# tzjtatata/Myriad

Hardware: AMD Instinct MI355X
Metric: images/sec fine-tune step (Vicuna-7B + LoRA-style adapters, 224px) (higher is better)
Workload: dtype bf16

## Files before the change

### include/myriad_hip.h

```cpp
#ifndef MYRIAD_HIP_H
#define MYRIAD_HIP_H
#include <stdint.h>

#ifdef __cplusplus
extern "C" {
#endif

typedef struct ihipStream_t* mh_stream_t;

#define MH_OK 0
#define MH_ERR_ARG (-1)
#define MH_ERR_LAUNCH (-2)
#define MH_ERR_UNSUPPORTED (-3)

#define MH_GEMM_OUT_F32 1
#define MH_GEMM_GELU 2
#define MH_GEMM_REGSTAGE 4

int mh_gemm_bf16_nt(const void* A, int lda, const void* B, int ldb, void* C, int ldc, int M, int N, int K,
                    const float* bias, const float* residual, int ldr, int flags, float alpha, mh_stream_t s);

int mh_gemm_plan(int M, int N, int K, int flags, int* kernel, int* splits);

int mh_prof_start(int capacity, mh_stream_t s);
// ... 120 lines not shown

int mh_clamp_ce(const float* logits, long ldl, const long* labels, float* row_loss, void* dlogits_bf16, long ldd,
                int R, int V, float grad_scale, mh_stream_t s);
int mh_sum_f32(const float* x, float* out, long n, float scale, mh_stream_t s);
int mh_argmax_rows(const float* logits, long ldl, long* out, float* margin, int R, int V, int ban_id, mh_stream_t s);
int mh_argmax_pmax_rows(const float* logits, long ldl, long* out, float* margin, float* pmax, int R, int V, int ban_id,
                        float inv_temp, mh_stream_t s);
int mh_decode_record(const long* nxt, const float* margin, const float* pmax, float* rec, long* next_ids, int* step, int R,
                     mh_stream_t s);
int mh_decode_advance(const long* nxt, const float* margin, const float* pmax, float* rec, long* next_ids, int* step, int* pos,
                      int* kvlen, int R, mh_stream_t s);
int mh_sample_rows(const float* logits, long ldl, long* out, float* margin, float* pmax, int* kept, float* u_out, int R, int V,
                   int ban_id, const float* params, const unsigned long long* seed, const int* step, int t_add, mh_stream_t s);
int mh_repetition_penalty_rows(float* logits, long ldl, unsigned* seen, const long* prev_ids, int R, int V, const float* penalty,
                               mh_stream_t s);
int mh_decode_advance_kept(const long* nxt, const float* margin, const float* pmax, const int* kept, float* rec, long* next_ids,
                           int* step, int* pos, int* kvlen, int R, mh_stream_t s);
int mh_decode_advance_rows(const long* nxt, const float* margin, const float* pmax, float* rec, long* next_ids, int* step,
                           int* pos, int* kvlen, const int* live, int R, mh_stream_t s);
int mh_sample_rows_slots(const float* logits, long ldl, long* out, float* margin, float* pmax, int* kept, float* u_out, int R, int V,
                         const float* params, const unsigned long long* seed, const int* gen, const int* live, mh_stream_t s);
int mh_argmax_pmax_rows_slots(const float* logits, long ldl, long* out, float* margin, float* pmax, int R, int V, const float* params,
                              const int* gen, const int* live, mh_stream_t s);
int mh_repetition_penalty_rows_slots(float* logits, long ldl, unsigned* seen, const long* prev_ids, int R, int V, const float* penalty,
                                     const int* live, mh_stream_t s);
int mh_decode_advance_kept_rows(const long* nxt, const float* margin, const float* pmax, const int* kept, float* rec, long* next_ids,
                                int* step, int* pos, int* kvlen, int* gen, const int* live, int R, mh_stream_t s);
int mh_token_scores_rows(const float* logits, long ldl, const long* ids, const int* watch, float* out, long ldo, int R, int V,
                         const int* live, mh_stream_t s);

int mh_beam_topk(const float* logits, long ldl, const float* scores, float* part_s, int* part_i, float* out_s, int* out_i, int B,
                 int rpi, int nb, int V, int ban_id, int* pos, int* kvlen, int n_adv, mh_stream_t s);
int mh_beam_reorder_kv(void* const* caches, int L, int B, int nb, long T_cap, int C, const int* src, const int* lo, const int* hi,
                       mh_stream_t s);
int mh_beam_topk_items(const float* logits, long ldl, const float* scores, float* part_s, int* part_i, float* out_s, int* out_i, int G,
                       int nb, int V, const int* live, int* gen, const int* prm, int* pos, int* kvlen, mh_stream_t s);
int mh_beam_reorder_kv_items(void* const* caches, int L, int G, int nb, long T_cap, int C, const int* src, const int* lo,
                             const int* hi, const int* live, mh_stream_t s);
int mh_beam_sample_topk(const float* logits, long ldl, const float* scores, const unsigned* seen, float* part_k, float* part_a,
                        int* part_i, int* part_f, float* out_s, int* out_i, int* out_f, float* out_k, int B, int nb, int V,
                        int ban_id, int draw, const float* params, const unsigned long long* seed, int* step, int t_add, int* pos,
                        int* kvlen, int n_adv, mh_stream_t s);
int mh_beam_seen_update(unsigned* seen, const int* src, const long* ids, int B, int nb, int V, mh_stream_t s);

int mh_im2col_nhwc(const void* x, void* col, int B, int H, int W, int C, int kh, int kw, int pad, int Kpad,
                   mh_stream_t s);
int mh_col2im_nhwc(const void* dcol, float* dx, int B, int H, int W, int C, int kh, int kw, int pad, int Kpad,
                   mh_stream_t s);
int mh_relu_maxpool2_fwd(const void* y, int y_is_f32, long ldy, void* p, int B, int H, int W, int C, mh_stream_t s);
int mh_relu_maxpool2_bwd(const float* dp, const void* y, int y_is_f32, long ldy, void* dy, long lddy, int B, int H,
                         int W, int C, mh_stream_t s);
int mh_conv_pack_weight(const float* W, const float* bias, void* Wp, int Cout, int K, int Kpad, mh_stream_t s);
int mh_conv_unpack_grad(const float* dWp, float* dW, float* db, int Cout, int K, int Kpad, mh_stream_t s);

int mh_embed_gather(const void* table_bf16, const long* ids, const int* dst_rows, float* out, long n, int D, long ldo,
                    mh_stream_t s);
int mh_copy2d_f32(const float* src, long lds, float* dst, long ldd, long rows, int cols, int accumulate,
                  mh_stream_t s);
int mh_copy3d_f32(const float* src, long src_bstride, long lds, float* dst, long dst_bstride, long ldd, int nb,
                  long rows, int cols, int accumulate, mh_stream_t s);
int mh_gather_rows_f32_to_bf16(const float* src, long lds, const int* rows, void* dst, long n, int D, mh_stream_t s);
int mh_gather_rows_f32(const float* src, long lds, const int* rows, float* dst, long n, int D, mh_stream_t s);
int mh_gather_rows(const void* src, long lds, const int* rows, void* dst, long n, int D, int elem_bytes, mh_stream_t s);
int mh_expand_rows(const void* src, const int* inv, void* dst, long ldd, long M, int D, int elem_bytes, mh_stream_t s);
int mh_copy3d_bf16(const void* src, long src_bstride, long lds, void* dst, long dst_bstride, long ldd, int nb,
                   long rows, int cols, mh_stream_t s);
int mh_kv_append_bf16(const void* src, long ld_src, void* cache, long cache_bstride, long ld_cache, const int* pos_dev,
                      int B, int cols, mh_stream_t s);
int mh_rope_kv_append(void* qkv, long ld, int n_heads, int head_dim, const int* pos, const float* cos_tab,
                      const float* sin_tab, void* cache, long cache_bstride, long ld_cache, const int* pos_dev, int B,
                      mh_stream_t s);
int mh_add_i32(int* x, int n, int delta, mh_stream_t s);
long mh_gemv_pack_elems(int N, int K);
int mh_gemv_pack(const void* W, int ldb, int N, int K, void* out, mh_stream_t s);
int mh_gemv_packed(const void* A, int lda, const void* P, void* C, int ldc, int M, int N, int K, const float* bias,
                   const float* residual, int ldr, int out_f32, float alpha, mh_stream_t s);
int mh_gemv_packed_rmsnorm(const float* H, long ldh, const float* norm_w, float eps, const void* P, void* C, int ldc, int M,
                           int N, int K, const float* bias, const float* residual, int ldr, int out_f32, float alpha,
                           mh_stream_t s);
int mh_gemv_packed_silu(const void* gu, long ldgu, const void* P, void* C, int ldc, int M, int N, int K, const float* bias,
                        const float* residual, int ldr, int out_f32, float alpha, mh_stream_t s);
long mh_gemv_pack_fp8_elems(int N, int K);
int mh_gemv_pack_fp8(const void* W, int ldb, int N, int K, void* q_out, float* scale_out, mh_stream_t s);
int mh_gemv_packed_fp8(const void* A, int lda, const void* Q, const float* scale, void* C, int ldc, int M, int N, int K,
                       const float* bias, const float* residual, int ldr, int out_f32, float alpha, mh_stream_t s);
int mh_gemv_packed_fp8_rmsnorm(const float* H, long ldh, const float* norm_w, float eps, const void* Q, const float* scale,
                               void* C, int ldc, int M, int N, int K, const float* bias, const float* residual, int ldr,
                               int out_f32, float alpha, mh_stream_t s);
int mh_gemv_packed_fp8_silu(const void* gu, long ldgu, const void* Q, const float* scale, void* C, int ldc, int M, int N, int K,
                            const float* bias, const float* residual, int ldr, int out_f32, float alpha, mh_stream_t s);
long mh_gemv_pack_fp4_elems(int N, int K);
long mh_gemv_pack_fp4_scale_elems(int N, int K);
int mh_gemv_pack_fp4(const void* W, int ldb, int N, int K, void* q_out, void* scale_out, mh_stream_t s);
int mh_gemv_packed_fp4(const void* A, int lda, const void* Q, const void* scale, void* C, int ldc, int M, int N, int K,
                       const float* bias, const float* residual, int ldr, int out_f32, float alpha, mh_stream_t s);
int mh_gemv_packed_fp4_rmsnorm(const float* H, long ldh, const float* norm_w, float eps, const void* Q, const void* scale,
                               void* C, int ldc, int M, int N, int K, const float* bias, const float* residual, int ldr,
                               int out_f32, float alpha, mh_stream_t s);
int mh_gemv_packed_fp4_silu(const void* gu, long ldgu, const void* Q, const void* scale, void* C, int ldc, int M, int N, int K,
                            const float* bias, const float* residual, int ldr, int out_f32, float alpha, mh_stream_t s);
int mh_gemv_packed_wide(const void* A, int lda, const void* P, void* C, int ldc, int M, int N, int K, const float* bias,
                        const float* residual, int ldr, int out_f32, float alpha, mh_stream_t s);
int mh_gemv_packed_fp8_wide(const void* A, int lda, const void* Q, const float* scale, void* C, int ldc, int M, int N, int K,
                            const float* bias, const float* residual, int ldr, int out_f32, float alpha, mh_stream_t s);
int mh_gemv_packed_fp4_wide(const void* A, int lda, const void* Q, const void* scale, void* C, int ldc, int M, int N, int K,
                            const float* bias, const float* residual, int ldr, int out_f32, float alpha, mh_stream_t s);
// ... 123 lines not shown
```

### myriad_amd/csrc/common.h

```cpp
#pragma once
#include <hip/hip_runtime.h>
#include <stdint.h>

#define MH_OK 0
#define MH_ERR_ARG (-1)
#define MH_ERR_LAUNCH (-2)
#define MH_ERR_UNSUPPORTED (-3)

typedef unsigned short bf16_t;
typedef __attribute__((ext_vector_type(8))) short short8_t;
typedef __attribute__((ext_vector_type(4))) short short4_t;
typedef __attribute__((ext_vector_type(4))) float float4_t;
typedef __attribute__((ext_vector_type(16))) float float16_t;

#define MH_CHECK_LAUNCH()                                   \
  do {                                                      \
    hipError_t e__ = hipGetLastError();                     \
    if (e__ != hipSuccess) return MH_ERR_LAUNCH;            \
  } while (0)

#define MH_MAX_ALT_WS 4
struct MhScratch {
  float* ws;
  size_t bytes;
  float* alt[MH_MAX_ALT_WS];
  hipStream_t alt_stream[MH_MAX_ALT_WS];
};
extern MhScratch g_default_scratch;
extern MhScratch* g_scratch;

enum MhOpt {
  MH_OPT_SLAB_BF16 = 0,
  MH_OPT_GEMM_SKINNY,
  MH_OPT_SWIGLU_FUSED,
  MH_OPT_GELU_FUSED,
  MH_OPT_ATTN_BWD_SPLIT,
  MH_OPT_GEMM_ZERO_PAD,
  MH_OPT_GEMM256_IMPL,
  MH_OPT_LORA_NORM_FUSED,
  MH_OPT_ATTN_FULL,
  MH_OPT_LORA_WGRAD_MFMA,
  MH_OPT_GEMM_SKIP_PAD,
  MH_OPT_GEMM_SPLIT_XCD,
  MH_OPT_COUNT
};
int mh_opt(int id);

extern bool g_mh_prof_on;
void mh_prof_pre(hipStream_t s, int kernel, int M, int N, int K, int splits, int flags);
void mh_prof_post(hipStream_t s);

__device__ __forceinline__ float bf2f(bf16_t h) { return __uint_as_float(((unsigned)h) << 16); }

typedef __bf16 mh_bf2_t __attribute__((ext_vector_type(2)));
typedef float mh_f2_t __attribute__((ext_vector_type(2)));
__device__ __forceinline__ bf16_t f2bf_sw(float f) {
  unsigned u = __float_as_uint(f);
  if ((u & 0x7fffffffu) > 0x7f800000u) return (bf16_t)((u >> 16) | 0x40);
  u += 0x7fffu + ((u >> 16) & 1u);
  return (bf16_t)(u >> 16);
}
__device__ __forceinline__ bf16_t f2bf(float f) {
  const __bf16 b = (__bf16)f;
  return (bf16_t)__builtin_bit_cast(unsigned short, b);
}
__device__ __forceinline__ unsigned pack_bf2(float lo, float hi) {
  const mh_f2_t v = {lo, hi};
  const mh_bf2_t b = __builtin_convertvector(v, mh_bf2_t);
  return __builtin_bit_cast(unsigned, b);
}

__device__ __forceinline__ unsigned dropout_hash(unsigned long long seed, unsigned long long idx) {
  unsigned h = (unsigned)idx * 0x9E3779B1u + ((unsigned)seed ^ ((unsigned)(idx >> 32) * 0x85EBCA77u));
  h ^= (unsigned)(seed >> 32) & 0x7FFFFFFFu;
  h ^= h >> 16;
  h *= 0x85EBCA6Bu;
  h ^= h >> 13;
  h *= 0xC2B2AE35u;
  h ^= h >> 16;
  return h;
}
__device__ __forceinline__ unsigned dropout_hash2(unsigned h) {
  h = (h ^ 0x68E31DA4u) * 0x2C1B3C6Du;
  return h ^ (h >> 15);
}
__device__ __forceinline__ float dropout_keep(unsigned long long seed, unsigned long long idx, float p, float inv_keep) {
  if (p <= 0.f) return 1.f;
  unsigned h = dropout_hash(seed, idx);
  if (seed >> 63) h = dropout_hash2(h);
  const float u = (float)(h >> 8) * (1.0f / 16777216.0f);
  return u >= p ? inv_keep : 0.f;
}
__device__ __forceinline__ void dropout_keep_pair(unsigned long long seed, unsigned long long idx, float p, float inv_keep,
                                                  float& k0, float& k1) {
  if (p <= 0.f) { k0 = k1 = 1.f; return; }
  const unsigned h = dropout_hash(seed, idx);
// ... 85 lines not shown
```

### myriad_amd/csrc/conv.hip

```cpp
#include "common.h"

#define CV_NT 256
static inline int cv_grid(long n) {
  long g = (n + CV_NT - 1) / CV_NT;
  if (g > 4096) g = 4096;
  if (g < 1) g = 1;
  return (int)g;
}

__global__ void im2col_kernel(const bf16_t* __restrict__ x, bf16_t* __restrict__ col, int B, int H, int W, int C,
                              int kh, int kw, int pad, int OH, int OW, int K, int Kpad) {
  const int groups = Kpad >> 2;
  const long total = (long)B * OH * OW * groups;
  for (long it = blockIdx.x * (long)blockDim.x + threadIdx.x; it < total; it += (long)gridDim.x * blockDim.x) {
    const long m = it / groups;
    const int k0 = (int)(it - m * groups) * 4;
    const int ox = (int)(m % OW);
    const int oy = (int)((m / OW) % OH);
    const int b = (int)(m / ((long)OW * OH));
    bf16_t v[4];
#pragma unroll
    for (int e = 0; e < 4; ++e) {
      const int k = k0 + e;
      bf16_t val = 0;
// ... 153 lines not shown
#pragma unroll
      for (int e = 0; e < 8; ++e) {
        const int k = k0 + e;
        v[e] = k < K ? Wt[(long)co * K + k] : (k == K && bias ? bias[co] : 0.f);
      }
    }
    uint4 pk;
    pk.x = pack_bf2(v[0], v[1]); pk.y = pack_bf2(v[2], v[3]); pk.z = pack_bf2(v[4], v[5]); pk.w = pack_bf2(v[6], v[7]);
    *reinterpret_cast<uint4*>(Wp + (long)co * Kpad + k0) = pk;
  }
}
__global__ void conv_unpack_kernel(const float* __restrict__ dWp, float* __restrict__ dW, float* __restrict__ db,
                                   int Cout, int K, int Kpad) {
  if ((K & 3) == 0) {
    const int qpr = K >> 2;
    const long total = (long)Cout * (qpr + 1);
    for (long it = blockIdx.x * (long)blockDim.x + threadIdx.x; it < total; it += (long)gridDim.x * blockDim.x) {
      const int co = (int)(it / (qpr + 1)), q = (int)(it - (long)co * (qpr + 1));
      if (q == qpr) {
        if (db) db[co] = dWp[(long)co * Kpad + K];
      } else {
        *reinterpret_cast<float4_t*>(dW + (long)co * K + q * 4) = *reinterpret_cast<const float4_t*>(dWp + (long)co * Kpad + q * 4);
      }
    }
    return;
  }
  const long total = (long)Cout * (K + 1);
  for (long it = blockIdx.x * (long)blockDim.x + threadIdx.x; it < total; it += (long)gridDim.x * blockDim.x) {
    const int co = (int)(it / (K + 1)), j = (int)(it - (long)co * (K + 1));
    if (j == K) {
      if (db) db[co] = dWp[(long)co * Kpad + K];
    } else {
      dW[(long)co * K + j] = dWp[(long)co * Kpad + j];
    }
  }
}

extern "C" int mh_conv_pack_weight(const float* W, const float* bias, void* Wp, int Cout, int K, int Kpad,
                                   hipStream_t stream) {
  if (Kpad < K + 1 || (Kpad & 7) != 0) return MH_ERR_ARG;
  hipLaunchKernelGGL(conv_pack_kernel, dim3(cv_grid((long)Cout * (Kpad / 8))), dim3(CV_NT), 0, stream, W, bias,
                     (bf16_t*)Wp, Cout, K, Kpad);
  MH_CHECK_LAUNCH();
  return MH_OK;
}
extern "C" int mh_conv_unpack_grad(const float* dWp, float* dW, float* db, int Cout, int K, int Kpad,
                                   hipStream_t stream) {
  if (Kpad < K + 1) return MH_ERR_ARG;
  hipLaunchKernelGGL(conv_unpack_kernel, dim3(cv_grid((K & 3) ? (long)Cout * (K + 1) : (long)Cout * (K / 4 + 1))), dim3(CV_NT), 0, stream, dWp, dW, db,
                     Cout, K, Kpad);
  MH_CHECK_LAUNCH();
  return MH_OK;
}
```

### myriad_amd/csrc/version.hip

```cpp
#include "common.h"
#include <stdlib.h>
#include <string.h>
extern "C" const char* mh_version(void) { return "myriad_hip 0.1 (gfx950)"; }
extern "C" int mh_target_arch(void) { return 950; }

struct MhOptEntry { const char* name; const char* env; int def; int value; };
static MhOptEntry g_opts[MH_OPT_COUNT] = {
    {"slab_bf16", "MYRIAD_SLAB_BF16", 1, -1},
    {"gemm_skinny", "MYRIAD_GEMM_SKINNY", 1, -1},
    {"swiglu_fused", "MYRIAD_SWIGLU_FUSED", 1, -1},
    {"gelu_fused", "MYRIAD_GELU_FUSED", 1, -1},
    {"attn_bwd_split", "MYRIAD_ATTN_BWD_SPLIT", 1, -1},
    {"gemm_zero_pad", "MYRIAD_GEMM_ZERO_PAD", 1, -1},
    {"gemm256_impl", "MYRIAD_GEMM256_IMPL", 1, -1},
    {"lora_norm_fused", "MYRIAD_LORA_NORM_FUSED", 1, -1},
    {"attn_full", "MYRIAD_ATTN_FULL", 1, -1},
    {"lora_wgrad_mfma", "MYRIAD_LORA_WGRAD_MFMA", 1, -1},
    {"gemm_skip_pad", "MYRIAD_GEMM_SKIP_PAD", 1, -1},
    {"gemm_split_xcd", "MYRIAD_GEMM_SPLIT_XCD", 1, -1},
};

int mh_opt(int id) {
  MhOptEntry& o = g_opts[id];
  if (o.value < 0) {
    const char* e = getenv(o.env);
    o.value = e ? (e[0] == '0' ? 0 : 1) : o.def;
  }
  return o.value;
}

static int find_opt(const char* name) {
  if (!name) return -1;
  for (int i = 0; i < MH_OPT_COUNT; ++i)
    if (!strcmp(name, g_opts[i].name)) return i;
  return -1;
}
extern "C" int mh_get_option(const char* name) {
  const int i = find_opt(name);
  return i < 0 ? MH_ERR_ARG : mh_opt(i);
}
extern "C" int mh_set_option(const char* name, int value) {
  const int i = find_opt(name);
  if (i < 0 || (value != 0 && value != 1)) return MH_ERR_ARG;
  const int prev = mh_opt(i);
  g_opts[i].value = value;
  return prev;
}
```

### myriad_amd/networks.py

```python
from __future__ import annotations

from typing import Dict, List, Optional, Tuple

import torch

from . import ops

BF16, F32 = torch.bfloat16, torch.float32

STEM_CH = [(1, 4), (4, 16), (16, 64), (64, 256), (256, 1024)]
STEM_IDX = (0, 3, 6, 9, 12)


def ve_param_specs(prefix: str, head_out: int, head_k: int) -> List[Tuple[str, Tuple[int, ...], Tuple[int, ...]]]:
    specs = []
    for idx, (ci, co) in zip(STEM_IDX, STEM_CH):
        specs.append((f"{prefix}meta_net.{idx}.weight", (co, 9 * ci), (co, ci, 3, 3)))
        specs.append((f"{prefix}meta_net.{idx}.bias", (co,), (co,)))
    specs.append((f"{prefix}meta_net.15.weight", (head_out, head_k * head_k * 1024), (head_out, 1024, head_k, head_k)))
    specs.append((f"{prefix}meta_net.15.bias", (head_out,), (head_out,)))
    return specs


def from_reference_layout(t: torch.Tensor, internal_shape) -> torch.Tensor:
    if t.dim() == 4 and len(internal_shape) != 4:
        return t.permute(0, 2, 3, 1).reshape(internal_shape).contiguous()
    return t.reshape(internal_shape).contiguous()


def to_reference_layout(t: torch.Tensor, ref_shape) -> torch.Tensor:
    if len(ref_shape) == 4 and t.dim() != 4:
        co, ci, kh, kw = ref_shape
        return t.reshape(co, kh, kw, ci).permute(0, 3, 1, 2).contiguous()
    return t.reshape(ref_shape).contiguous()


class VENet:

    def __init__(self, prefix: str, head_k: int, head_out: int, params: Dict[str, torch.Tensor],
                 grads: Dict[str, torch.Tensor], device):
        self.prefix, self.head_k, self.head_out = prefix, head_k, head_out
        self.p, self.g, self.dev = params, grads, torch.device(device)
        self._saved = None

    def _w(self, idx):
        return self.p[f"{self.prefix}meta_net.{idx}.weight"], self.p[f"{self.prefix}meta_net.{idx}.bias"]

    def forward(self, maps: torch.Tensor, save_for_backward: bool = True) -> torch.Tensor:
        B, _, H, W = maps.shape
        x = ops.to_bf16(maps.contiguous()).view(B, H, W, 1)
        saved = []
        for idx, (ci, co) in zip(STEM_IDX, STEM_CH):
            wm, bias = self._w(idx)
            wp = ops.conv_pack(wm, bias)
            col = ops.im2col(x, 3, 3, 1)
            y = ops.gemm(col, wp, out_dtype=F32)
            saved.append((col, y, wp, H, W, ci, co))
            x = ops.relu_pool_fwd(y, B, H, W, co)
            H, W = H // 2, W // 2
        wm, bias = self._w(15)
        if self.head_k == 1:
            x2 = x.view(B * H * W, 1024)
            wb = ops.to_bf16(wm)
            out = ops.gemm(x2, wb, bias=bias, out_dtype=F32)
            head = (x2, wb, None, True)
            T = H * W
        else:
            k = self.head_k
            T = (H - k + 1) * (W - k + 1)
            if wm.shape[1] % 64 == 0:
                wp = ops.to_bf16(wm)
                col = ops.im2col(x, k, k, 0, bias_col=False)
                out = ops.gemm(col, wp, bias=bias, out_dtype=F32)
                head = (col, wp, (H, W), True)
            else:
                wp = ops.conv_pack(wm, bias)
                col = ops.im2col(x, k, k, 0)
                out = ops.gemm(col, wp, out_dtype=F32)
                head = (col, wp, (H, W), False)
        if save_for_backward:
            self._saved = dict(stem=saved, head=head, B=B)
        return out.view(B, T, self.head_out)

    @property
    def head_accumulates_in_place(self) -> bool:
        return self.head_k != 1 and (self.head_k * self.head_k * 1024) % 64 == 0

    def backward(self, dtokens: torch.Tensor, accumulate_head: bool = False) -> None:
        sv = self._saved
        if sv is None:
            raise RuntimeError("backward() without saved forward")
        B = sv["B"]
        dy32 = dtokens.reshape(-1, self.head_out).contiguous()
        dyb = ops.to_bf16(dy32)
        gw, gb = self.g[f"{self.prefix}meta_net.15.weight"], self.g[f"{self.prefix}meta_net.15.bias"]
        a, wq, hw = sv["head"][:3]
        dyT = ops.transpose_to_bf16(dyb, 64)
        if self.head_k == 1:
            ops.gemm_auto_f32(dyT, ops.transpose_to_bf16(a, 64), gw)
            gb.copy_(ops.colsum(dy32))
            dp = ops.gemm(dyb, ops.transpose_to_bf16(wq, 64), out_dtype=F32)
        else:
            Kpad = wq.shape[1]
            if sv["head"][3]:
                if accumulate_head:
                    ops.gemm(dyT, ops.transpose_to_bf16(a, 64), out=gw, residual=gw)
                else:
                    ops.gemm_auto_f32(dyT, ops.transpose_to_bf16(a, 64), gw)
                gb.copy_(ops.colsum(dy32))
            else:
                dwp = torch.empty((self.head_out, Kpad), dtype=F32, device=self.dev)
                ops.gemm_auto_f32(dyT, ops.transpose_to_bf16(a, 64), dwp)
                ops.conv_unpack_grad(dwp, gw, gb)
            dcol = ops.gemm(dyb, ops.transpose_to_bf16(wq, 64))
            H, W = hw
            dp = ops.col2im(dcol, B, H, W, 1024, self.head_k, self.head_k, 0)
        for li in range(4, -1, -1):
            col, y, wp, H, W, ci, co = sv["stem"][li]
            idx = STEM_IDX[li]
            dy, dyfull = ops.relu_pool_bwd(dp, y, B, H, W, co, pad_cols_to=64)
            dwp = torch.empty((co, wp.shape[1]), dtype=F32, device=self.dev)
            ops.gemm_auto_f32(ops.transpose_to_bf16(dy, 64), ops.transpose_to_bf16(col, 64), dwp)
            ops.conv_unpack_grad(dwp, self.g[f"{self.prefix}meta_net.{idx}.weight"],
                                 self.g[f"{self.prefix}meta_net.{idx}.bias"])
            if li > 0:
                wpT = ops.transpose_to_bf16(wp, 64)
                dcol = ops.gemm(dyfull, wpT)
                dp = ops.col2im(dcol, B, H, W, ci, 3, 3, 1)
        self._saved = None


class LoraAdaptor:

    def __init__(self, params, grads, prefix="expert_adaptor."):
        self.A, self.Bm = params[prefix + "conv1.weight"], params[prefix + "conv2.weight"]
        self.gA, self.gB = grads[prefix + "conv1.weight"], grads[prefix + "conv2.weight"]
        self._saved = None

    def forward(self, x2d: torch.Tensor, save_for_backward=True):
        y, t = ops.lowrank_fwd(x2d, self.A, self.Bm)
        if save_for_backward:
            self._saved = (x2d, t)
        return y

    def backward(self, dy2d: torch.Tensor, need_dx: bool = False):
        x2d, t = self._saved
        dx = ops.lowrank_bwd(dy2d, x2d, t, self.A, self.Bm, self.gA, self.gB, need_dx=need_dx)
        self._saved = None
        return dx
```

### myriad_amd/ops.py

```python
from __future__ import annotations

import math
import numbers
from typing import Optional

import os

import torch

from . import _lib

BF16 = torch.bfloat16
F32 = torch.float32

GEMM_OUT_F32 = 1
GEMM_GELU = 2
GEMM_REGSTAGE = 4
GEMM_VARIANT = 0


def _L():
    return _lib.load()


# ... 1282 lines not shown
    _chk_flat(src, torch.int32, B * nb, "beam_seen_update: src")
    _chk_flat(ids, torch.long, B * nb, "beam_seen_update: ids")
    _lib.check(_L().mh_beam_seen_update(_p(seen), _p(src), _p(ids), B, nb, V, _s()), "mh_beam_seen_update")
    return seen


def im2col(x_nhwc: torch.Tensor, kh: int, kw: int, pad: int, bias_col: bool = True):
    B, H, W, C = x_nhwc.shape
    OH, OW = H + 2 * pad - kh + 1, W + 2 * pad - kw + 1
    Kpad = round_up(kh * kw * C + (1 if bias_col else 0), 64)
    if not bias_col and Kpad != kh * kw * C:
        raise _lib.MyriadHipError(f"im2col: bias_col=False needs kh*kw*C % 64 == 0, got {kh * kw * C}")
    col = torch.empty((B * OH * OW, Kpad), dtype=BF16, device=x_nhwc.device)
    _lib.check(_L().mh_im2col_nhwc(_p(x_nhwc), _p(col), B, H, W, C, kh, kw, pad, Kpad, _s()), "mh_im2col_nhwc")
    return col


def col2im(dcol: torch.Tensor, B, H, W, C, kh, kw, pad):
    dx = torch.empty((B, H, W, C), dtype=F32, device=dcol.device)
    _lib.check(_L().mh_col2im_nhwc(_p(dcol), _p(dx), B, H, W, C, kh, kw, pad, dcol.stride(0), _s()), "mh_col2im_nhwc")
    return dx


def relu_pool_fwd(y2d: torch.Tensor, B, H, W, C):
    p = torch.empty((B, H // 2, W // 2, C), dtype=BF16, device=y2d.device)
    _lib.check(_L().mh_relu_maxpool2_fwd(_p(y2d), int(y2d.dtype == F32), y2d.stride(0), _p(p), B, H, W, C, _s()),
               "mh_relu_maxpool2_fwd")
    return p


def relu_pool_bwd(dp: torch.Tensor, y2d: torch.Tensor, B, H, W, C, pad_cols_to: int = 1):
    cpad = round_up(C, pad_cols_to)
    full = (torch.zeros if cpad != C else torch.empty)((B * H * W, cpad), dtype=BF16, device=y2d.device)
    _lib.check(_L().mh_relu_maxpool2_bwd(_p(dp), _p(y2d), int(y2d.dtype == F32), y2d.stride(0), _p(full),
                                         full.stride(0), B, H, W, C, _s()), "mh_relu_maxpool2_bwd")
    return full[:, :C], full


def conv_pack(Wm: torch.Tensor, bias: Optional[torch.Tensor], out=None):
    Cout, K = Wm.shape
    Kpad = round_up(K + 1, 64)
    if out is None:
        out = torch.empty((Cout, Kpad), dtype=BF16, device=Wm.device)
    _lib.check(_L().mh_conv_pack_weight(_p(Wm), _p(bias), _p(out), Cout, K, Kpad, _s()), "mh_conv_pack_weight")
    return out


def conv_unpack_grad(dWp: torch.Tensor, dW: torch.Tensor, db: Optional[torch.Tensor]):
    Cout, Kpad = dWp.shape
    K = dW.shape[1]
    _lib.check(_L().mh_conv_unpack_grad(_p(dWp), _p(dW), _p(db), Cout, K, Kpad, _s()), "mh_conv_unpack_grad")


def adamw_step(p, g, m, v, lr, wd, step, beta1=0.9, beta2=0.999, eps=1e-8, grad_scale=1.0, shadow=None):
    _lib.check(_L().mh_adamw_step(_p(p), _p(g), _p(m), _p(v), _p(shadow), p.numel(), float(lr), float(beta1),
                                  float(beta2), float(eps), float(wd), int(step), float(grad_scale), _s()),
               "mh_adamw_step")


def adamw_gated(p, g, m, v, lr, wd, used: torch.Tensor, steps: torch.Tensor, beta1=0.9, beta2=0.999, eps=1e-8, grad_scale=1.0):
    _lib.check(_L().mh_adamw_gated(_p(p), _p(g), _p(m), _p(v), p.numel(), float(lr), float(beta1), float(beta2), float(eps),
                                   float(wd), float(grad_scale), _p(used), _p(steps), _s()), "mh_adamw_gated")


def adamw_bump(used: torch.Tensor, steps: torch.Tensor):
    _lib.check(_L().mh_adamw_bump(_p(used), _p(steps), steps.numel(), _s()), "mh_adamw_bump")


def grad_sumsq_slots(n: int) -> int:
    return int(_L().mh_grad_sumsq_slots(int(n)))


def grad_sumsq(g: torch.Tensor, used: torch.Tensor, partials: torch.Tensor) -> int:
    _lib.check(_L().mh_grad_sumsq(_p(g), g.numel(), _p(used), _p(partials), partials.numel(), _s()), "mh_grad_sumsq")
    return grad_sumsq_slots(g.numel())


def clip_rank_sum(partials: torch.Tensor, n_partials: int, rank_sums: torch.Tensor, rank: int):
    _lib.check(_L().mh_clip_rank_sum(_p(partials), int(n_partials), _p(rank_sums), rank_sums.numel(), int(rank), _s()),
               "mh_clip_rank_sum")


def clip_finalize(partials: torch.Tensor, n_partials: int, rank_sums: Optional[torch.Tensor], max_norm: Optional[float],
                  grad_scale: float, guard: bool, ctl: torch.Tensor):
    if n_partials > partials.numel() or ctl.numel() < 4 or ctl.dtype != torch.float64 or partials.dtype != torch.float64:
        raise _lib.MyriadHipError("clip_finalize: f64 partials / ctl[4] expected")
    _lib.check(_L().mh_clip_finalize(_p(partials), int(n_partials), _p(rank_sums), 0 if rank_sums is None else rank_sums.numel(),
                                     float("inf") if max_norm is None else float(max_norm), float(grad_scale), int(bool(guard)),
                                     _p(ctl), _s()), "mh_clip_finalize")


def adamw_gated_ctl(p, g, m, v, lr, wd, used: torch.Tensor, steps: torch.Tensor, ctl: torch.Tensor, beta1=0.9, beta2=0.999, eps=1e-8):
    _lib.check(_L().mh_adamw_gated_ctl(_p(p), _p(g), _p(m), _p(v), p.numel(), float(lr), float(beta1), float(beta2), float(eps),
                                       float(wd), _p(used), _p(steps), _p(ctl), _s()), "mh_adamw_gated_ctl")


def adamw_bump_ctl(used: torch.Tensor, steps: torch.Tensor, ctl: torch.Tensor):
    _lib.check(_L().mh_adamw_bump_ctl(_p(used), _p(steps), steps.numel(), _p(ctl), _s()), "mh_adamw_bump_ctl")


def l2norm_rows(x: torch.Tensor, want_bf16: bool = True, want_f32: bool = False, eps: float = 1e-12):
    _chk2d(x, F32, "l2norm_rows.x")
    M, D = x.shape
    yb = torch.empty((M, D), dtype=BF16, device=x.device) if want_bf16 else None
    yf = torch.empty((M, D), dtype=F32, device=x.device) if want_f32 else None
    _lib.check(_L().mh_l2norm_rows(_p(x), x.stride(0), _p(yb), _p(yf), D, M, D, float(eps), _s()), "mh_l2norm_rows")
# ... 166 lines not shown
```

Baseline: 206.4.

## Add direct fused conv3x3+ReLU+maxpool kernels for thin vision-encoder stem layers

Replaces the im2col+GEMM path for the thin stem convolutions (Ci up to 16) with a direct kernel that fuses conv, ReLU and 2x2 max-pool and records the pooled argmax as a route byte. Matching direct weight-gradient (two-stage partial+reduce) and data-gradient kernels consume that route, skipping the im2col buffers, padded GEMMs and relu_pool backward passes. Larger stem layers and the head switch their weight gradients to a TN wgrad GEMM, removing transposes. The change adds several custom kernels and shape restrictions, and rounding must match the bf16 GEMM path. The vision encoder is a small part of a 7B LLM step.

Result: no change. 207.6 (median of 6 runs) (+0.6%).

```diff
diff --git a/include/myriad_hip.h b/include/myriad_hip.h
--- a/include/myriad_hip.h
+++ b/include/myriad_hip.h
@@ -196,6 +196,13 @@
                          int W, int C, mh_stream_t s);
 int mh_conv_pack_weight(const float* W, const float* bias, void* Wp, int Cout, int K, int Kpad, mh_stream_t s);
 int mh_conv_unpack_grad(const float* dWp, float* dW, float* db, int Cout, int K, int Kpad, mh_stream_t s);
+int mh_conv3x3_relu_pool_fwd(const void* x, const float* W, const float* bias, void* p, void* route, int B, int H, int Wd,
+                             int Ci, int Co, mh_stream_t s);
+long mh_conv3x3_wgrad_ws_floats(int B, int H, int Wd, int Ci, int Co);
+int mh_conv3x3_wgrad(const float* dp, const void* route, const void* x, float* dW, float* db, float* ws, long ws_floats, int B,
+                     int H, int Wd, int Ci, int Co, mh_stream_t s);
+int mh_conv3x3_dgrad(const float* dp, const void* route, const float* W, float* dx, int B, int H, int Wd, int Ci, int Co,
+                     mh_stream_t s);
 
 int mh_embed_gather(const void* table_bf16, const long* ids, const int* dst_rows, float* out, long n, int D, long ldo,
                     mh_stream_t s);
diff --git a/myriad_amd/csrc/common.h b/myriad_amd/csrc/common.h
--- a/myriad_amd/csrc/common.h
+++ b/myriad_amd/csrc/common.h
@@ -42,6 +42,7 @@
   MH_OPT_LORA_WGRAD_MFMA,
   MH_OPT_GEMM_SKIP_PAD,
   MH_OPT_GEMM_SPLIT_XCD,
+  MH_OPT_VE_DIRECT_CONV,
   MH_OPT_COUNT
 };
 int mh_opt(int id);
diff --git a/myriad_amd/csrc/conv.hip b/myriad_amd/csrc/conv.hip
--- a/myriad_amd/csrc/conv.hip
+++ b/myriad_amd/csrc/conv.hip
@@ -229,3 +229,344 @@
   MH_CHECK_LAUNCH();
   return MH_OK;
 }
+
+#define CV_ROUTE_NONE 4
+#define CV_WG_MAXT 576
+#define CV_WG_UNROLL 4
+#define CV_WG_RL 16
+
+__device__ __forceinline__ float cv_round_bf16(float v) { return bf2f(f2bf(v)); }
+
+template <int CI, int COG>
+__global__ __launch_bounds__(CV_NT) void conv3x3_relu_pool_fwd_kernel(const bf16_t* __restrict__ x, const float* __restrict__ Wt,
+                                                                      const float* __restrict__ bias, bf16_t* __restrict__ p,
+                                                                      unsigned char* __restrict__ route, int B, int H, int W,
+                                                                      int CO) {
+  constexpr int CC = CI < 4 ? CI : 4;
+  constexpr int K = 9 * CI;
+  __shared__ float sw[K * COG + COG];
+  const int co0 = blockIdx.y * COG;
+  for (int i = threadIdx.x; i < K * COG; i += CV_NT) {
+    const int k = i / COG, j = i - k * COG;
+    sw[i] = cv_round_bf16(Wt[(long)(co0 + j) * K + k]);
+  }
+  if (threadIdx.x < COG) sw[K * COG + threadIdx.x] = cv_round_bf16(bias[co0 + threadIdx.x]);
+  __syncthreads();
+  const int PH = H >> 1, PW = W >> 1;
+  const long total = (long)B * PH * PW;
+  const long q = blockIdx.x * (long)CV_NT + threadIdx.x;
+  if (q < total) {
+    const int px = (int)(q % PW);
+    const int py = (int)((q / PW) % PH);
+    const int b = (int)(q / ((long)PW * PH));
+    float acc[4][COG];
+#pragma unroll
+    for (int e = 0; e < 4; ++e)
+#pragma unroll
+      for (int j = 0; j < COG; ++j) acc[e][j] = sw[K * COG + j];
+#pragma unroll 1
+    for (int c0 = 0; c0 < CI; c0 += CC) {
+      float patch[4][4][CC];
+#pragma unroll
+      for (int dy = 0; dy < 4; ++dy) {
+        const int iy = 2 * py - 1 + dy;
+#pragma unroll
+        for (int dx = 0; dx < 4; ++dx) {
+          const int ix = 2 * px - 1 + dx;
+          const bool in = iy >= 0 && iy < H && ix >= 0 && ix < W;
+          const bf16_t* src = x + (((long)b * H + iy) * W + ix) * CI + c0;
+          if (CC == 4) {
+            uint2 v = {0u, 0u};
+            if (in) v = *reinterpret_cast<const uint2*>(src);
+            patch[dy][dx][0] = __uint_as_float(v.x << 16);
+            patch[dy][dx][1 % CC] = __uint_as_float(v.x & 0xFFFF0000u);
+            patch[dy][dx][2 % CC] = __uint_as_float(v.y << 16);
+            patch[dy][dx][3 % CC] = __uint_as_float(v.y & 0xFFFF0000u);
+          } else {
+#pragma unroll
+            for (int c = 0; c < CC; ++c) patch[dy][dx][c] = in ? bf2f(src[c]) : 0.f;
+          }
+        }
+      }
+#pragma unroll
+      for (int ky = 0; ky < 3; ++ky)
+#pragma unroll
+        for (int kx = 0; kx < 3; ++kx)
+#pragma unroll
+          for (int c = 0; c < CC; ++c) {
+            const float* wk = sw + ((ky * 3 + kx) * CI + c0 + c) * COG;
+#pragma unroll
+            for (int j = 0; j < COG; ++j) {
+              const float w = wk[j];
+#pragma unroll
+              for (int e = 0; e < 4; ++e) acc[e][j] = __builtin_fmaf(patch[(e >> 1) + ky][(e & 1) + kx][c], w, acc[e][j]);
+            }
+          }
+    }
+    bf16_t pv[COG];
+    unsigned char rv[COG];
+#pragma unroll
+    for (int j = 0; j < COG; ++j) {
+      float best = acc[0][j];
+      int arg = 0;
+#pragma unroll
+      for (int e = 1; e < 4; ++e)
+        if (acc[e][j] > best) { best = acc[e][j]; arg = e; }
+      float m = 0.f;
+#pragma unroll
+      for (int e = 0; e < 4; ++e) m = fmaxf(m, acc[e][j]);
+      pv[j] = f2bf(m);
+      rv[j] = (unsigned char)(best > 0.f ? arg : CV_ROUTE_NONE);
+    }
+    const long o = q * CO + co0;
+#pragma unroll
+    for (int j = 0; j < COG; j += 4) {
+      uint2 pk;
+      pk.x = (unsigned)pv[j] | ((unsigned)pv[j + 1] << 16);
+      pk.y = (unsigned)pv[j + 2] | ((unsigned)pv[j + 3] << 16);
+      *reinterpret_cast<uint2*>(p + o + j) = pk;
+      *reinterpret_cast<unsigned*>(route + o + j) =
+          (unsigned)rv[j] | ((unsigned)rv[j + 1] << 8) | ((unsigned)rv[j + 2] << 16) | ((unsigned)rv[j + 3] << 24);
+    }
+  }
+}
+
+static inline bool cv_direct_shape_ok(int B, int H, int W, int Ci, int Co) {
+  if (!(B > 0 && H >= 2 && W >= 2 && !(H & 1) && !(W & 1) && (Ci == 1 || Ci == 4 || Ci == 16) && Co >= 4 && Co <= 64 && !(Co & 3)))
+    return false;
+  return (long)B * H * W * (Ci > Co ? Ci : Co) < 0x7FFFFFFFL;
+}
+
+template <int CI>
+static int cv_fwd_launch(const void* x, const float* Wt, const float* bias, void* p, void* route, int B, int H, int W, int Co,
+                         hipStream_t stream) {
+  const long total = (long)B * (H / 2) * (W / 2);
+  if ((total + CV_NT - 1) / CV_NT > 0x7FFFFFFFL) return MH_ERR_UNSUPPORTED;
+  const int gx = (int)((total + CV_NT - 1) / CV_NT);
+  hipLaunchKernelGGL((conv3x3_relu_pool_fwd_kernel<CI, 4>), dim3(gx, Co / 4), dim3(CV_NT), 0, stream, (const bf16_t*)x, Wt, bias,
+                     (bf16_t*)p, (unsigned char*)route, B, H, W, Co);
+  MH_CHECK_LAUNCH();
+  return MH_OK;
+}
+
+extern "C" int mh_conv3x3_relu_pool_fwd(const void* x, const float* Wt, const float* bias, void* p, void* route, int B, int H,
+                                        int W, int Ci, int Co, hipStream_t stream) {
+  if (!x || !Wt || !bias || !p || !route || B <= 0 || H <= 0 || W <= 0 || Ci <= 0 || Co <= 0) return MH_ERR_ARG;
+  if (!cv_direct_shape_ok(B, H, W, Ci, Co)) return MH_ERR_UNSUPPORTED;
+  if (Ci == 1) return cv_fwd_launch<1>(x, Wt, bias, p, route, B, H, W, Co, stream);
+  if (Ci == 4) return cv_fwd_launch<4>(x, Wt, bias, p, route, B, H, W, Co, stream);
+  return cv_fwd_launch<16>(x, Wt, bias, p, route, B, H, W, Co, stream);
+}
+
+template <int CI>
+__global__ __launch_bounds__(CV_WG_MAXT) void conv3x3_wgrad_partial_kernel(const float* __restrict__ dp,
+                                                                           const unsigned char* __restrict__ route,
+                                                                           const bf16_t* __restrict__ x, float* __restrict__ part,
+                                                                           int B, int H, int W, int CO, int PL, int per) {
+  extern __shared__ float red[];
+  const int owners = CO * 9;
+  const int l = threadIdx.x / owners, o = threadIdx.x - l * owners;
+  const int co = o / 9, tap = o - co * 9;
+  const int ky = tap / 3, kx = tap - ky * 3;
+  const int PH = H >> 1, PW = W >> 1;
+  const int Q = B * PH * PW;
+  const int q0 = blockIdx.x * per;
+  const int q1 = q0 + per < Q ? q0 + per : Q;
+  float acc[CI];
+#pragma unroll
+  for (int c = 0; c < CI; ++c) acc[c] = 0.f;
+  float accb = 0.f;
+  for (int qb = q0 + l; qb < q1; qb += PL * CV_WG_UNROLL) {
+    int r[CV_WG_UNROLL], qq[CV_WG_UNROLL];
+    float g[CV_WG_UNROLL];
+#pragma unroll
+    for (int u = 0; u < CV_WG_UNROLL; ++u) {
+      const int q = qb + u * PL;
+      qq[u] = q < q1 ? q : q0;
+      r[u] = route[(long)qq[u] * CO + co];
+      g[u] = dp[(long)qq[u] * CO + co];
+    }
+#pragma unroll
+    for (int u = 0; u < CV_WG_UNROLL; ++u) {
+      const bool live = qb + u * PL < q1 && r[u] < CV_ROUTE_NONE;
+      const float gu = live ? cv_round_bf16(g[u]) : 0.f;
+      const int ru = live ? r[u] : 0;
+      const int px = qq[u] % PW;
+      const int t = qq[u] / PW;
+      const int py = t % PH, b = t / PH;
+      const int iy = 2 * py + (ru >> 1) + ky - 1, ix = 2 * px + (ru & 1) + kx - 1;
+      const bool in = iy >= 0 && iy < H && ix >= 0 && ix < W;
+      const bf16_t* src = x + (((long)b * H + (in ? iy : 0)) * W + (in ? ix : 0)) * CI;
+      if (tap == 4) accb += gu;
+      if (CI >= 4) {
+#pragma unroll
+        for (int c = 0; c < CI; c += 4) {
+          uint2 v = *reinterpret_cast<const uint2*>(src + c);
+          if (!in) v = make_uint2(0u, 0u);
+          acc[c] = __builtin_fmaf(gu, __uint_as_float(v.x << 16), acc[c]);
+          acc[(c + 1) % CI] = __builtin_fmaf(gu, __uint_as_float(v.x & 0xFFFF0000u), acc[(c + 1) % CI]);
+          acc[(c + 2) % CI] = __builtin_fmaf(gu, __uint_as_float(v.y << 16), acc[(c + 2) % CI]);
+          acc[(c + 3) % CI] = __builtin_fmaf(gu, __uint_as_float(v.y & 0xFFFF0000u), acc[(c + 3) % CI]);
+        }
+      } else {
+#pragma unroll
+        for (int c = 0; c < CI; ++c) acc[c] = __builtin_fmaf(gu, in ? bf2f(src[c]) : 0.f, acc[c]);
+      }
+    }
+  }
+  if (PL > 1) {
+    float* mine = red + ((long)l * owners + o) * (CI + 1);
+#pragma unroll
+    for (int c = 0; c < CI; ++c) mine[c] = acc[c];
+    mine[CI] = accb;
+    __syncthreads();
+    if (l == 0) {
+      for (int k = 1; k < PL; ++k) {
+        const float* other = red + ((long)k * owners + o) * (CI + 1);
+#pragma unroll
+        for (int c = 0; c < CI; ++c) acc[c] += other[c];
+        accb += other[CI];
+      }
+    }
+  }
+  if (l == 0) {
+    const long nout = (long)CO * 9 * CI + CO;
+    float* dst = part + blockIdx.x * nout;
+#pragma unroll
+    for (int c = 0; c < CI; ++c) dst[(long)o * CI + c] = acc[c];
+    if (tap == 4) dst[(long)CO * 9 * CI + co] = accb;
+  }
+}
+
+__global__ __launch_bounds__(CV_NT) void conv3x3_wgrad_reduce_kernel(const float* __restrict__ part, float* __restrict__ dW,
+                                                                     float* __restrict__ db, int nW, int nB, int nchunk) {
+  __shared__ float red[CV_NT];
+  const int lane = threadIdx.x / (CV_NT / CV_WG_RL), jj = threadIdx.x - lane * (CV_NT / CV_WG_RL);
+  const int j = blockIdx.x * (CV_NT / CV_WG_RL) + jj;
+  float s = 0.f;
+  if (j < nW + nB)
+    for (int k = lane; k < nchunk; k += CV_WG_RL) s += part[(long)k * (nW + nB) + j];
+  red[threadIdx.x] = s;
+  __syncthreads();
+  if (lane == 0 && j < nW + nB) {
+    for (int i = 1; i < CV_WG_RL; ++i) s += red[i * (CV_NT / CV_WG_RL) + jj];
+    if (j < nW) dW[j] = s;
+    else if (db) db[j - nW] = s;
+  }
+}
+
+static void cv_wgrad_plan(int B, int H, int W, int Ci, int Co, int* PL, int* per, int* nchunk) {
+  const int Q = B * (H / 2) * (W / 2);
+  int pl = CV_WG_MAXT / (Co * 9);
+  if (pl > 16) pl = 16;
+  if (pl < 1) pl = 1;
+  if (pl > Q) pl = Q;
+  const int cap = Co * 9 * Ci + Co > 4096 ? 256 : 1024;
+  int n = (Q + pl * 8 - 1) / (pl * 8);
+  if (n > cap) n = cap;
+  const int pp = (Q + n - 1) / n;
+  *PL = pl;
+  *per = pp;
+  *nchunk = (Q + pp - 1) / pp;
+}
+
+extern "C" long mh_conv3x3_wgrad_ws_floats(int B, int H, int W, int Ci, int Co) {
+  if (!cv_direct_shape_ok(B, H, W, Ci, Co)) return MH_ERR_UNSUPPORTED;
+  int PL, nchunk, per;
+  cv_wgrad_plan(B, H, W, Ci, Co, &PL, &per, &nchunk);
+  return (long)nchunk * ((long)Co * 9 * Ci + Co);
+}
+
+extern "C" int mh_conv3x3_wgrad(const float* dp, const void* route, const void* x, float* dW, float* db, float* ws,
+                                long ws_floats, int B, int H, int W, int Ci, int Co, hipStream_t stream) {
+  if (!dp || !route || !x || !dW || !ws || B <= 0 || H <= 0 || W <= 0 || Ci <= 0 || Co <= 0) return MH_ERR_ARG;
+  if (!cv_direct_shape_ok(B, H, W, Ci, Co)) return MH_ERR_UNSUPPORTED;
+  int PL, nchunk, per;
+  cv_wgrad_plan(B, H, W, Ci, Co, &PL, &per, &nchunk);
+  const int nW = Co * 9 * Ci, nB = Co;
+  if (ws_floats < (long)nchunk * (nW + nB)) return MH_ERR_ARG;
+  const dim3 grid(nchunk), block(Co * 9 * PL);
+  const size_t lds = PL > 1 ? (size_t)PL * Co * 9 * (Ci + 1) * sizeof(float) : 0;
+  const unsigned char* rt = (const unsigned char*)route;
+  if (Ci == 1)
+    hipLaunchKernelGGL(conv3x3_wgrad_partial_kernel<1>, grid, block, lds, stream, dp, rt, (const bf16_t*)x, ws, B, H, W, Co, PL, per);
+  else if (Ci == 4)
+    hipLaunchKernelGGL(conv3x3_wgrad_partial_kernel<4>, grid, block, lds, stream, dp, rt, (const bf16_t*)x, ws, B, H, W, Co, PL, per);
+  else
+    hipLaunchKernelGGL(conv3x3_wgrad_partial_kernel<16>, grid, block, lds, stream, dp, rt, (const bf16_t*)x, ws, B, H, W, Co, PL, per);
+  MH_CHECK_LAUNCH();
+  const int opb = CV_NT / CV_WG_RL;
+  hipLaunchKernelGGL(conv3x3_wgrad_reduce_kernel, dim3((nW + nB + opb - 1) / opb), dim3(CV_NT), 0, stream, ws, dW, db, nW, nB,
+                     nchunk);
+  MH_CHECK_LAUNCH();
+  return MH_OK;
+}
+
+template <int CI>
+__global__ __launch_bounds__(CV_NT) void conv3x3_dgrad_kernel(const float* __restrict__ dp, const unsigned char* __restrict__ route,
+                                                              const float* __restrict__ Wt, float* __restrict__ dx, int B, int H,
+                                                              int W, int CO) {
+  constexpr int CG = CI < 4 ? CI : 4;
+  constexpr int NG = CI / CG;
+  extern __shared__ float sw[];
+  for (int i = threadIdx.x; i < CO * 9 * CI; i += CV_NT) sw[i] = cv_round_bf16(Wt[i]);
+  __syncthreads();
+  const int PH = H >> 1, PW = W >> 1;
+  const int total = B * H * W * NG;
+  for (int it = blockIdx.x * CV_NT + threadIdx.x; it < total; it += gridDim.x * CV_NT) {
+    const int cg = it % NG;
+    const int pix = it / NG;
+    const int ix = pix % W;
+    const int t = pix / W;
+    const int iy = t % H, b = t / H;
+    float acc[CG];
+#pragma unroll
+    for (int c = 0; c < CG; ++c) acc[c] = 0.f;
+    const int py0 = ((iy + 1) >> 1) - 1, px0 = ((ix + 1) >> 1) - 1;
+    for (int a = 0; a < 4; ++a) {
+      const int py = py0 + (a >> 1), px = px0 + (a & 1);
+      if (py < 0 || py >= PH || px < 0 || px >= PW) continue;
+      const long q = ((long)b * PH + py) * PW + px;
+      const int dyc = iy + 1 - 2 * py, dxc = ix + 1 - 2 * px;
+#pragma unroll 4
+      for (int co4 = 0; co4 < CO; co4 += 4) {
+        const unsigned rr = *reinterpret_cast<const unsigned*>(route + q * CO + co4);
+        const float4_t gg = *reinterpret_cast<const float4_t*>(dp + q * CO + co4);
+#pragma unroll
+        for (int j = 0; j < 4; ++j) {
+          const int r = (int)((rr >> (8 * j)) & 0xFFu);
+          const int ky = dyc - ((r >> 1) & 1), kx = dxc - (r & 1);
+          const bool hit = r < CV_ROUTE_NONE && ky >= 0 && ky < 3 && kx >= 0 && kx < 3;
+          const float g = hit ? cv_round_bf16(gg[j]) : 0.f;
+          const float* w = sw + ((co4 + j) * 9 + (hit ? ky * 3 + kx : 0)) * CI + cg * CG;
+#pragma unroll
+          for (int c = 0; c < CG; ++c) acc[c] = __builtin_fmaf(g, w[c], acc[c]);
+        }
+      }
+    }
+    float* dst = dx + (long)pix * CI + cg * CG;
+    if (CG == 4) {
+      *reinterpret_cast<float4_t*>(dst) = (float4_t){acc[0], acc[1 % CG], acc[2 % CG], acc[3 % CG]};
+    } else {
+#pragma unroll
+      for (int c = 0; c < CG; ++c) dst[c] = acc[c];
+    }
+  }
+}
+
+extern "C" int mh_conv3x3_dgrad(const float* dp, const void* route, const float* Wt, float* dx, int B, int H, int W, int Ci,
+                                int Co, hipStream_t stream) {
+  if (!dp || !route || !Wt || !dx || B <= 0 || H <= 0 || W <= 0 || Ci <= 0 || Co <= 0) return MH_ERR_ARG;
+  if (!cv_direct_shape_ok(B, H, W, Ci, Co)) return MH_ERR_UNSUPPORTED;
+  const size_t lds = (size_t)Co * 9 * Ci * sizeof(float);
+  const unsigned char* rt = (const unsigned char*)route;
+  const dim3 block(CV_NT);
+  if (Ci == 1)
+    hipLaunchKernelGGL(conv3x3_dgrad_kernel<1>, dim3(cv_grid((long)B * H * W)), block, lds, stream, dp, rt, Wt, dx, B, H, W, Co);
+  else if (Ci == 4)
+    hipLaunchKernelGGL(conv3x3_dgrad_kernel<4>, dim3(cv_grid((long)B * H * W)), block, lds, stream, dp, rt, Wt, dx, B, H, W, Co);
+  else
+    hipLaunchKernelGGL(conv3x3_dgrad_kernel<16>, dim3(cv_grid((long)B * H * W * 4)), block, lds, stream, dp, rt, Wt, dx, B, H, W, Co);
+  MH_CHECK_LAUNCH();
+  return MH_OK;
+}
diff --git a/myriad_amd/csrc/version.hip b/myriad_amd/csrc/version.hip
--- a/myriad_amd/csrc/version.hip
+++ b/myriad_amd/csrc/version.hip
@@ -18,6 +18,7 @@
     {"lora_wgrad_mfma", "MYRIAD_LORA_WGRAD_MFMA", 1, -1},
     {"gemm_skip_pad", "MYRIAD_GEMM_SKIP_PAD", 1, -1},
     {"gemm_split_xcd", "MYRIAD_GEMM_SPLIT_XCD", 1, -1},
+    {"ve_direct_conv", "MYRIAD_VE_DIRECT_CONV", 1, -1},
 };
 
 int mh_opt(int id) {
diff --git a/myriad_amd/networks.py b/myriad_amd/networks.py
--- a/myriad_amd/networks.py
+++ b/myriad_amd/networks.py
@@ -10,6 +10,7 @@
 
 STEM_CH = [(1, 4), (4, 16), (16, 64), (64, 256), (256, 1024)]
 STEM_IDX = (0, 3, 6, 9, 12)
+THIN_MAX_CI = 16
 
 
 def ve_param_specs(prefix: str, head_out: int, head_k: int) -> List[Tuple[str, Tuple[int, ...], Tuple[int, ...]]]:
@@ -49,9 +50,16 @@
     def forward(self, maps: torch.Tensor, save_for_backward: bool = True) -> torch.Tensor:
         B, _, H, W = maps.shape
         x = ops.to_bf16(maps.contiguous()).view(B, H, W, 1)
+        direct = ops.ve_direct_conv()
         saved = []
         for idx, (ci, co) in zip(STEM_IDX, STEM_CH):
             wm, bias = self._w(idx)
+            if direct and ci <= THIN_MAX_CI:
+                p, route = ops.conv3x3_relu_pool_fwd(x, wm, bias)
+                saved.append((x, route, None, H, W, ci, co))
+                x = p
+                H, W = H // 2, W // 2
+                continue
             wp = ops.conv_pack(wm, bias)
             col = ops.im2col(x, 3, 3, 1)
             y = ops.gemm(col, wp, out_dtype=F32)
@@ -79,7 +87,7 @@
                 out = ops.gemm(col, wp, out_dtype=F32)
                 head = (col, wp, (H, W), False)
         if save_for_backward:
-            self._saved = dict(stem=saved, head=head, B=B)
+            self._saved = dict(stem=saved, head=head, B=B, direct=direct)
         return out.view(B, T, self.head_out)
 
     @property
@@ -95,9 +103,13 @@
         dyb = ops.to_bf16(dy32)
         gw, gb = self.g[f"{self.prefix}meta_net.15.weight"], self.g[f"{self.prefix}meta_net.15.bias"]
         a, wq, hw = sv["head"][:3]
-        dyT = ops.transpose_to_bf16(dyb, 64)
+        direct = sv["direct"]
+        dyT = None if direct and self.head_k == 1 else ops.transpose_to_bf16(dyb, 64)
         if self.head_k == 1:
-            ops.gemm_auto_f32(dyT, ops.transpose_to_bf16(a, 64), gw)
+            if direct:
+                ops.gemm_tn_wgrad(dyb, a, gw)
+            else:
+                ops.gemm_auto_f32(dyT, ops.transpose_to_bf16(a, 64), gw)
             gb.copy_(ops.colsum(dy32))
             dp = ops.gemm(dyb, ops.transpose_to_bf16(wq, 64), out_dtype=F32)
         else:
@@ -118,11 +130,19 @@
         for li in range(4, -1, -1):
             col, y, wp, H, W, ci, co = sv["stem"][li]
             idx = STEM_IDX[li]
+            gw, gb = self.g[f"{self.prefix}meta_net.{idx}.weight"], self.g[f"{self.prefix}meta_net.{idx}.bias"]
+            if wp is None:
+                ops.conv3x3_wgrad(dp, y, col, gw, gb)
+                if li > 0:
+                    dp = ops.conv3x3_dgrad(dp, y, self._w(idx)[0], B, H, W)
+                continue
             dy, dyfull = ops.relu_pool_bwd(dp, y, B, H, W, co, pad_cols_to=64)
-            dwp = torch.empty((co, wp.shape[1]), dtype=F32, device=self.dev)
-            ops.gemm_auto_f32(ops.transpose_to_bf16(dy, 64), ops.transpose_to_bf16(col, 64), dwp)
-            ops.conv_unpack_grad(dwp, self.g[f"{self.prefix}meta_net.{idx}.weight"],
-                                 self.g[f"{self.prefix}meta_net.{idx}.bias"])
+            if direct:
+                ops.gemm_tn_wgrad(dy, col[:, :9 * ci], gw, bias=gb)
+            else:
+                dwp = torch.empty((co, wp.shape[1]), dtype=F32, device=self.dev)
+                ops.gemm_auto_f32(ops.transpose_to_bf16(dy, 64), ops.transpose_to_bf16(col, 64), dwp)
+                ops.conv_unpack_grad(dwp, gw, gb)
             if li > 0:
                 wpT = ops.transpose_to_bf16(wp, 64)
                 dcol = ops.gemm(dyfull, wpT)
diff --git a/myriad_amd/ops.py b/myriad_amd/ops.py
--- a/myriad_amd/ops.py
+++ b/myriad_amd/ops.py
@@ -1358,6 +1358,52 @@
     _lib.check(_L().mh_conv_unpack_grad(_p(dWp), _p(dW), _p(db), Cout, K, Kpad, _s()), "mh_conv_unpack_grad")
 
 
+def ve_direct_conv() -> bool:
+    return _L().mh_get_option(b"ve_direct_conv") == 1
+
+
+def conv3x3_relu_pool_fwd(x_nhwc: torch.Tensor, Wm: torch.Tensor, bias: torch.Tensor):
+    B, H, W, Ci = x_nhwc.shape
+    Co = Wm.shape[0]
+    if x_nhwc.dtype != BF16 or not x_nhwc.is_contiguous() or Wm.dtype != F32 or tuple(Wm.shape) != (Co, 9 * Ci) \
+            or not Wm.is_contiguous() or bias.dtype != F32 or bias.numel() != Co or not bias.is_contiguous():
+        raise ValueError(f"conv3x3_relu_pool_fwd: x {tuple(x_nhwc.shape)} {x_nhwc.dtype} W {tuple(Wm.shape)} bias {tuple(bias.shape)}")
+    p = torch.empty((B, H // 2, W // 2, Co), dtype=BF16, device=x_nhwc.device)
+    route = torch.empty((B, H // 2, W // 2, Co), dtype=torch.uint8, device=x_nhwc.device)
+    _lib.check(_L().mh_conv3x3_relu_pool_fwd(_p(x_nhwc), _p(Wm), _p(bias), _p(p), _p(route), B, H, W, Ci, Co, _s()),
+               f"mh_conv3x3_relu_pool_fwd B={B} H={H} W={W} Ci={Ci} Co={Co}")
+    return p, route
+
+
+def conv3x3_wgrad(dp: torch.Tensor, route: torch.Tensor, x_nhwc: torch.Tensor, dW: torch.Tensor, db: Optional[torch.Tensor]):
+    B, H, W, Ci = x_nhwc.shape
+    Co = dW.shape[0]
+    if dp.dtype != F32 or not dp.is_contiguous() or dp.numel() != route.numel() or route.dtype != torch.uint8 \
+            or tuple(route.shape) != (B, H // 2, W // 2, Co) or not route.is_contiguous() or not x_nhwc.is_contiguous() \
+            or dW.dtype != F32 or tuple(dW.shape) != (Co, 9 * Ci) or not dW.is_contiguous() \
+            or (db is not None and (db.dtype != F32 or db.numel() != Co or not db.is_contiguous())):
+        raise ValueError(f"conv3x3_wgrad: dp {tuple(dp.shape)} route {tuple(route.shape)} x {tuple(x_nhwc.shape)} dW {tuple(dW.shape)}")
+    L = _L()
+    n = L.mh_conv3x3_wgrad_ws_floats(B, H, W, Ci, Co)
+    if n < 0:
+        _lib.check(int(n), f"mh_conv3x3_wgrad_ws_floats B={B} H={H} W={W} Ci={Ci} Co={Co}")
+    ws = torch.empty((n,), dtype=F32, device=dp.device)
+    _lib.check(L.mh_conv3x3_wgrad(_p(dp), _p(route), _p(x_nhwc), _p(dW), _p(db), _p(ws), n, B, H, W, Ci, Co, _s()),
+               f"mh_conv3x3_wgrad B={B} H={H} W={W} Ci={Ci} Co={Co}")
+
+
+def conv3x3_dgrad(dp: torch.Tensor, route: torch.Tensor, Wm: torch.Tensor, B, H, W):
+    Co, K = Wm.shape
+    Ci = K // 9
+    if dp.dtype != F32 or not dp.is_contiguous() or route.dtype != torch.uint8 or not route.is_contiguous() \
+            or tuple(route.shape) != (B, H // 2, W // 2, Co) or dp.numel() != route.numel() or Wm.dtype != F32 or not Wm.is_contiguous():
+        raise ValueError(f"conv3x3_dgrad: dp {tuple(dp.shape)} route {tuple(route.shape)} W {tuple(Wm.shape)}")
+    dx = torch.empty((B, H, W, Ci), dtype=F32, device=dp.device)
+    _lib.check(_L().mh_conv3x3_dgrad(_p(dp), _p(route), _p(Wm), _p(dx), B, H, W, Ci, Co, _s()),
+               f"mh_conv3x3_dgrad B={B} H={H} W={W} Ci={Ci} Co={Co}")
+    return dx
+
+
 def adamw_step(p, g, m, v, lr, wd, step, beta1=0.9, beta2=0.999, eps=1e-8, grad_scale=1.0, shadow=None):
     _lib.check(_L().mh_adamw_step(_p(p), _p(g), _p(m), _p(v), _p(shadow), p.numel(), float(lr), float(beta1),
                                   float(beta2), float(eps), float(wd), int(step), float(grad_scale), _s()),
```
